# Prayforhanluo/HiCHap_master

Hardware: AMD Instinct MI355X
Metric: ICE iterations/sec on 10 kb whole-genome matrix (also nnz*iters/sec) (higher is better)
Workload: dtype f64; 1 GPU; hg19-10kb-diploid-wholegenome; n_bins=607282, nnz_upper=4998527599, resolution_bp=10000, parallelism=single GPU, entries_stored=9997055198, slots_u32=160483740, slots_u16=3332512024, payload_bytes=14837255808, tiles=88993, units=88985, hbm_bytes_matrix=15785038153

## Files before the change

hichap_master_amd/_lib.py:

```python
from __future__ import annotations

import ctypes as C
import os

_HERE = os.path.dirname(os.path.abspath(__file__))
LIB_PATH = os.environ.get("HH_LIB") or os.path.join(_HERE, "libhichap_hip.so")

HH_OK = 0


class HipLibraryError(RuntimeError):

    def __init__(self, code, msg):
        super().__init__(f"[hh rc={code}] {msg}")
        self.code = code


class MatrixInfo(C.Structure):
    _fields_ = [(n, C.c_int64) for n in (
        "n_bins", "row_lo", "row_hi", "nnz_upper", "n_entries", "n_slots", "n_tiles",
        "n_units", "n_wide", "device_bytes", "n_slots_narrow", "payload_bytes")] + [
        (n, C.c_int32) for n in ("n_chroms", "ignore_diags", "cis_only", "device", "band_w", "n_units_flat")] + [
        ("n_band", C.c_int64), ("payload_bytes_flat", C.c_int64)] + [
        (n, C.c_int32) for n in ("band_w4", "upper")]
# ... 31 lines not shown
    "hh_ktime_query": (C.c_int, [C.c_char_p, P, P]),
    "hh_ktime_reset": (C.c_int, []),
    "hh_matrix_from_pixels": (C.c_int, [P, P, P, I64, I64, P, I32, I32, I32, I64, I64, P, C.POINTER(P)]),
    "hh_matrix_from_pixels_device": (C.c_int, [P, P, P, I64, I64, P, I32, I32, I32, I64, I64, P, C.POINTER(P)]),
    "hh_matrix_free": (C.c_int, [P]),
    "hh_matrix_get_info": (C.c_int, [P, C.POINTER(MatrixInfo)]),
    "hh_matrix_export_upper": (C.c_int, [P, P, P, P, PI64]),
    "hh_synth_count": (C.c_int, [C.POINTER(SynthParams), P, P, P]),
    "hh_synth_build": (C.c_int, [C.POINTER(SynthParams), I64, I64, P, C.POINTER(P)]),
    "hh_synth_dense": (C.c_int, [P, I32, P, P]),
    "hh_synth_pixels": (C.c_int, [C.POINTER(SynthParams), I32, P, C.POINTER(P)]),
    "hh_pixels_get": (C.c_int, [P, P, P, P, PI64]),
    "hh_pixels_free": (C.c_int, [P]),
    "hh_ice_balance": (C.c_int, [P, C.POINTER(IceOpts), P, P, P, P, P, PF64, P]),
    "hh_ice_create": (C.c_int, [P, C.POINTER(IceOpts), C.POINTER(P)]),
    "hh_ice_free": (C.c_int, [P]),
    "hh_ice_n_groups": (C.c_int, [P, PI32]),
    "hh_ice_marg_local": (C.c_int, [P, I32, P, P]),
    "hh_ice_set_marg": (C.c_int, [P, P, I32, I64, P, P]),
    "hh_ice_filter_nnz": (C.c_int, [P, P]),
    "hh_ice_filter_count_mad": (C.c_int, [P, P]),
    "hh_ice_update": (C.c_int, [P, P]),
    "hh_ice_active_groups": (C.c_int, [P, PI32, P]),
    "hh_ice_iterations_done": (C.c_int, [P, PI32]),
    "hh_ice_run": (C.c_int, [P, I32, P]),
    "hh_ice_finalize": (C.c_int, [P, P, P, P, P, P, P]),
    "hh_ice_last_sweep_timing": (C.c_int, [P, PF64, PI32, PF64]),
    "hh_ice_swept_bytes": (C.c_int, [P, PI64]),
    "hh_ice_get_bias": (C.c_int, [P, P, P]),
    "hh_ice_set_bias": (C.c_int, [P, P, P]),
    "hh_ice_uband_fallbacks": (C.c_int, [P, PI64, P]),
    "hh_sweep_trace": (C.c_int, [P, I64, PI64]),
    "hh_matrix_stream_probe": (C.c_int, [P, I32, PF64, I32]),
    "hh_comm_unique_id": (C.c_int, [P]),
    "hh_comm_init": (C.c_int, [P, I32, I32, C.POINTER(P)]),
    "hh_comm_free": (C.c_int, [P]),
    "hh_comm_allgather": (C.c_int, [P, I64, P, P, P]),
    "hh_comm_reduce_scatter": (C.c_int, [P, I64, P, P, P]),
    "hh_ice_set_column_exchange": (C.c_int, [P, I32, I32, P, P, P, P, P]),
    "hh_ice_balance_sharded": (C.c_int, [P, C.POINTER(IceOpts), I32, I32, P, P, P, P, P, P, P, P, PF64, P]),
    "hh_ice_balance_cis_local": (C.c_int, [P, C.POINTER(IceOpts), I32, I64, P, P, P, P, P, P, P, PF64, P]),
    "hh_ice_filters_sharded": (C.c_int, [P, I32, P, P, P, P]),
    "hh_ice_run_sharded": (C.c_int, [P, I32, P, P, P, I32, P]),
    "hh_dense_rowstats": (C.c_int, [P, I32, I64, P, P, P, P, I32, P]),
    "hh_dense_symvc": (C.c_int, [P, I32, I64, P, P, F64, F64, P, I32, P]),
    "hh_twostep": (C.c_int, [P, P, P, I64, P, P, P, P, I32, P]),
    "hh_twostep_batch": (C.c_int, [I32, P, P, P, P, P, P, P, P, I32, P]),
    "hh_dense_from_cells": (C.c_int, [P, P, P, I64, I64, I64, I32, I32, P, P]),
    "hh_dense_upper_count": (C.c_int, [P, I64, PI64, P]),
    "hh_dense_upper_write": (C.c_int, [P, I64, P, P, P, P]),
    "hh_comp_create": (C.c_int, [P, I64, I32, P, C.POINTER(P)]),
    "hh_comp_free": (C.c_int, [P]),
    "hh_comp_colnnz": (C.c_int, [P, P, P]),
    "hh_comp_diag_sums": (C.c_int, [P, P, P, P]),
    "hh_comp_sliding_oe": (C.c_int, [P, P, I32, P]),
    "hh_comp_get_sliding_oe": (C.c_int, [P, P, P]),
    "hh_comp_correlation": (C.c_int, [P, P, P, I64, P]),
    "hh_comp_get_cor": (C.c_int, [P, P, P]),
    "hh_comp_set_cor": (C.c_int, [P, P, P]),
    "hh_gap_scan": (C.c_int, [P, I64, I32, I32, P, I32, P]),
    "hh_di_scan": (C.c_int, [P, I64, I32, P, P, I32, P, I32, P]),
    "hh_band_from_pixels": (C.c_int, [P, P, P, I64, P, I64, I64, I64, I32, P, I32, P]),
    "hh_tad_scan_pixels": (C.c_int, [P, P, P, I64, P, I64, I64, I64, I32, P, I32, P, P, I32, P]),
    "hh_viterbi_gmm": (C.c_int, [P, I64, I32, I32, P, P, P, P, P, P, P]),
    "hh_hmm_bw_create": (C.c_int, [P, P, I64, I32, I32, P, C.POINTER(P)]),
    "hh_hmm_bw_free": (C.c_int, [P]),
# ... 112 lines not shown
```

hichap_master_amd/csrc/ice.hip:

```cpp
#include <algorithm>
#include <chrono>
#include <functional>
#include <cmath>
#include <limits>

#include "ice_internal.hpp"

namespace hh {
constexpr int kThreads = 256;

constexpr int kSweepThreads = 512;
constexpr int kSweepWaves = kSweepThreads / 64;
constexpr int kFlatU = 8;
static_assert(kFlatU == kFlatIlvU, "k_sweep_flatw walks the interleaved layout's runs");

__device__ __forceinline__ double lds_b(const double* bl, uint32_t byteoff) {
    return *reinterpret_cast<const double*>(reinterpret_cast<const char*>(bl) + byteoff);
}

__device__ __forceinline__ void tile_dot(const uint4 v, const double* __restrict__ bl, double& a0, double& a1) {
    const uint32_t w[4] = {v.x, v.y, v.z, v.w};
    double x[4];
#pragma unroll
    for (int i = 0; i < 4; ++i) x[i] = lds_b(bl, w[i] & 0xFFFFu);
// ... 904 lines not shown
            flat_seg<UW, ABL, 4, true>(payw4, vw, qaw, qbw, i0w, i1w, fstw, fidw, nfw, bl, acc, lane, ca);
        } else {
            flat_seg_c<U, ABL, 8>(payn4, v, qan, qbn, i0n, i1n, fstn, nfn, bl, accc, lane);
            flat_seg<UW, ABL, 4>(payw4, vw, qaw, qbw, i0w, i1w, fstw, fidw, nfw, bl, acc, lane);
        }
        if (defer) {
            nfn_prev = nfn;
            fidn_prev = reinterpret_cast<const uint16_t*>(rg) + 2 * (kR + 1);
        } else {
            __syncthreads();
            for (int k = threadIdx.x; k < nfn; k += kSweepThreads) acc[fidn[k]] += accc[k];
        }
    }
    __syncthreads();
    for (int k = threadIdx.x; k < nfn_prev; k += kSweepThreads) acc[fidn_prev[k]] += accc[k];
    if (UP && cslot >= 0) flush_cols(L.cacc, T.colpart + (size_t)cslot * kW, kSweepThreads);
    __syncthreads();
    for (int k = threadIdx.x; k < nr; k += kSweepThreads) part[T.u_slot[u] + k] = acc[k];
}

template <int U, int ABL, bool UP>
__global__ __launch_bounds__(kSweepThreads, 4) void k_sweep_flat(TileDev T, const uint8_t* __restrict__ act,
                                                               int n_list, int list_off,
                                                               const double* __restrict__ b, long long n_bins,
                                                               double* __restrict__ part) {
    __shared__ __attribute__((aligned(16))) FlatLds<UP> L;
    if ((int)blockIdx.x >= n_list) return;
    sweep_flat_unit<U, ABL, UP>(T, act, T.u_order[list_off + blockIdx.x], b, n_bins, part, L);
}


template <int NW, bool UP>
struct FlatWLds {
    double bl[kW];
    u64 cacc[UP ? kW : 1];
    uint16_t rec[NW][kFrecU4 * 8];
    double acc[NW][kR];
    int next;
};

__device__ __forceinline__ void wave_lds_sync() {
    __builtin_amdgcn_fence(__ATOMIC_RELEASE, "wavefront");
    __builtin_amdgcn_wave_barrier();
    __builtin_amdgcn_fence(__ATOMIC_ACQUIRE, "wavefront");
}


template <int U, int ABL, int PIPE = 2, int NW = kFlatWaves, bool UP = false>
__global__ __launch_bounds__(NW * 64, NW > 8 ? 3 : 2) void k_sweep_flatw(TileDev T, const uint8_t* __restrict__ act,
                                                                       const double* __restrict__ b, long long n_bins,
                                                                       double* __restrict__ part) {
    constexpr int UW = 2;
    __shared__ __attribute__((aligned(16))) FlatWLds<NW, UP> L;
    const int k0 = T.fg_ptr[blockIdx.x], nk = T.fg_ptr[blockIdx.x + 1] - k0;
    {
        bool on = false;
        for (int k = 0; k < nk && !on; ++k) {
            const int u = T.fg_unit[k0 + k];
            for (int g = T.u_glo[u]; g <= T.u_ghi[u]; ++g) on |= act[g] != 0;
        }
        if (!on) return;
    }
    const int wave = __builtin_amdgcn_readfirstlane(threadIdx.x >> 6), lane = threadIdx.x & 63;
    const int J = T.tile_J[T.u_tlo[T.fg_unit[k0]]];
    const FlatDesc* __restrict__ desc = T.fg_desc + k0;
    const int cslot = UP && T.upper ? T.fg_cslot[blockIdx.x] : -1;
    if (threadIdx.x == 0) L.next = 0;
    if (ABL != 2 && threadIdx.x < kSweepThreads) stage_bias(L.bl, b, (long long)J * kW, n_bins);
    if (cslot >= 0)
        for (int k = threadIdx.x; k < kW; k += NW * 64) L.cacc[k] = 0;
    __syncthreads();
    const double* __restrict__ bl = L.bl;
    uint16_t* __restrict__ rec = L.rec[wave];
    double* __restrict__ acc = L.acc[wave];
    const uint16_t* fstn = rec;
    const uint16_t* fstw = rec + (kR + 1);
    const uint16_t* fidn = rec + 2 * (kR + 1);
    const uint16_t* fidw = fidn + kR;
    struct Tw {
        int slot, frec, nr, nfn, nfw;
        uint32_t qbn, qbw;
        const uint4 *payn4, *payw4;
        int up;
        const u64* bblk;
    };
    auto grab = [&](Tw& x) -> bool {
        for (;;) {
            int k = 0;
            if (lane == 0) k = atomicAdd(&L.next, 1);
            k = __builtin_amdgcn_readfirstlane(__shfl(k, 0, 64));
            if (k >= nk) return false;
            const FlatDesc d = desc[k];
            bool on = false;
            const int ngr = d.ghi - d.glo + 1;
            if (ngr <= 64) {
                const uint8_t a = act[d.glo + (lane < ngr ? lane : ngr - 1)];
                on = __ballot((a != 0) & (lane < ngr)) != 0;
            } else {
                for (int g = d.glo; g <= d.ghi; ++g) on |= act[g] != 0;
            }
            if (!on) continue;
            x = Tw{d.slot, d.frec, (int)d.nr, (int)d.nfn, (int)d.nfw, d.qbn, d.qbw,
                   reinterpret_cast<const uint4*>(T.payn + d.entn), reinterpret_cast<const uint4*>(T.pay + d.ent),
                   cslot >= 0 && d.upper ? 1 : 0, T.bfix + T.row_lo + (long long)d.rb * kR};
            return true;
        }
    };
    Tw cur;
    const bool any = grab(cur);
    uint4 v[U], vw[UW];
    if (any && cur.nfn) flat_load_ilv<U>(cur.payn4, 0u, cur.qbn, lane, v);
    if (any && cur.nfw) flat_load<UW>(cur.payw4, (uint32_t)lane * UW, 0u, cur.qbw, vw);
    for (; any;) {
        const uint4* rg = T.frec + (size_t)cur.frec * kFrecU4;
        const bool idn = cur.nfn == cur.nr;
        {
            static_assert((kR + 1 + 7) / 8 + 1 <= 2 * 64, "record range > 2 uint4 per lane");
            uint4* r4 = reinterpret_cast<uint4*>(rec);
            const int h0[4] = {0, kR + 1, 2 * (kR + 1), 2 * (kR + 1) + kR};
            const int h1[4] = {cur.nfn + 1, kR + 1 + cur.nfw + 1, idn ? 2 * (kR + 1) : 2 * (kR + 1) + cur.nfn,
                               2 * (kR + 1) + kR + cur.nfw};
            uint4 tq[4][2];
            int qs[4][2];
#pragma unroll
            for (int g = 0; g < 4; ++g) {
                const int q0 = h0[g] / 8, q1 = (h1[g] + 7) / 8;
#pragma unroll
                for (int h = 0; h < 2; ++h) {
                    const int q = q0 + lane + 64 * h;
                    qs[g][h] = q < q1 ? q : q0;
                    tq[g][h] = rg[qs[g][h]];
                }
            }
#pragma unroll
            for (int g = 0; g < 4; ++g)
#pragma unroll
                for (int h = 0; h < 2; ++h) r4[qs[g][h]] = tq[g][h];
        }
        wave_lds_sync();
        const ColArgs ca{cur.bblk, L.cacc};
        if (UP && cur.up) {
            flat_seg_c<U, ABL, 8, true, true>(cur.payn4, v, 0u, cur.qbn, 0, cur.nfn, fstn, cur.nfn, bl, acc, lane,
                                              ca, idn ? nullptr : fidn);
        } else {
            if (PIPE)
                flat_seg_c_pipe<U, ABL, 8, false, true>(cur.payn4, v, 0u, cur.qbn, 0, cur.nfn, fstn, cur.nfn, bl, acc,
                                                        lane);
            else
                flat_seg_c<U, ABL, 8, false, true>(cur.payn4, v, 0u, cur.qbn, 0, cur.nfn, fstn, cur.nfn, bl, acc, lane);
        }
        wave_lds_sync();
        constexpr int PL = kR / 64;
        double cv[PL];
        int cid[PL];
#pragma unroll
        for (int q = 0; q < PL; ++q) {
            const int i = lane + 64 * q;
            cv[q] = i < cur.nfn ? acc[i] : 0.0;
            cid[q] = i < cur.nfn ? (idn ? i : (int)fidn[i]) : -1;
        }
        wave_lds_sync();
#pragma unroll
        for (int q = 0; q < PL; ++q) acc[lane + 64 * q] = 0.0;
        wave_lds_sync();
#pragma unroll
        for (int q = 0; q < PL; ++q)
            if (cid[q] >= 0) acc[cid[q]] = cv[q];
        wave_lds_sync();
        if (UP && cur.up) {
            if (PIPE)
                flat_seg_pipe<UW, ABL, 4, true>(cur.payw4, vw, 0u, cur.qbw, 0, cur.nfw, fstw, fidw, cur.nfw, bl, acc, lane,
                                                ca);
            else flat_seg<UW, ABL, 4, true>(cur.payw4, vw, 0u, cur.qbw, 0, cur.nfw, fstw, fidw, cur.nfw, bl, acc, lane, ca);
        } else {
            if (PIPE) flat_seg_pipe<UW, ABL, 4>(cur.payw4, vw, 0u, cur.qbw, 0, cur.nfw, fstw, fidw, cur.nfw, bl, acc, lane);
            else flat_seg<UW, ABL, 4>(cur.payw4, vw, 0u, cur.qbw, 0, cur.nfw, fstw, fidw, cur.nfw, bl, acc, lane);
        }
        wave_lds_sync();
        Tw nxt;
        bool more = false;
        if (PIPE == 2) {
            more = grab(nxt);
            if (more) {
                if (nxt.nfn) flat_load_ilv<U>(nxt.payn4, 0u, nxt.qbn, lane, v);
                if (nxt.nfw) flat_load<UW>(nxt.payw4, (uint32_t)lane * UW, 0u, nxt.qbw, vw);
            }
        }
        double* __restrict__ out = part + cur.slot;
        for (int r = lane; r < cur.nr; r += 64) out[r] = acc[r];
        wave_lds_sync();
        if (PIPE != 2) {
            more = grab(nxt);
            if (more) {
                if (nxt.nfn) flat_load_ilv<U>(nxt.payn4, 0u, nxt.qbn, lane, v);
                if (nxt.nfw) flat_load<UW>(nxt.payw4, (uint32_t)lane * UW, 0u, nxt.qbw, vw);
            }
        }
        if (!more) break;
        cur = nxt;
    }
    if (UP && cslot >= 0) {
// ... 1169 lines not shown
    DBuf<unsigned long long> cx_send, cx_recv, cx_all;
    int32_t iters_done = 0;
    PinnedBuf<uint8_t> h_active;
    std::vector<hipEvent_t> ev;
    double sweep_ms = 0.0, iter_ms = 0.0;
    int32_t sweep_launches = 0;
    hipStream_t side = nullptr, side2 = nullptr;
    hipEvent_t fork = nullptr, join = nullptr, join2 = nullptr;
    ~hh_ice() {
        for (auto e : ev) (void)hipEventDestroy(e);
        if (join2) (void)hipEventDestroy(join2);
        if (side2) (void)hipStreamDestroy(side2);
        if (fork) (void)hipEventDestroy(fork);
        if (join) (void)hipEventDestroy(join);
        if (side) (void)hipStreamDestroy(side);
    }
    bool full() const { return m->row_lo == 0 && m->row_hi == m->n_bins; }
    TileArgs ta() {
        return TileArgs{tile_lo.p, tile_hi.p, tile_group.p, group_tile_ptr.p, blk_tile_ptr.p, tile_cnt.p,
                        tile_sum.p, tile_sq.p, g_cnt.p, g_sum.p, counter.p};
    }
    bool small_stats() const { return hh::g_fuse_stats == 1 || (hh::g_fuse_stats < 0 && n_tiles <= hh::kFuseMaxTiles); }
    uint8_t* act() { return active.p + (iters_done & 1) * G; }
    uint8_t* nxt() { return active.p + (1 - (iters_done & 1)) * G; }
};

namespace hh {

static int g_sweep_nb = 2;
static int g_band_dpp = 0;
static int g_flatw_waves = 11;
static int g_flatw_waves_up = 8;
static int g_flatw_pipe = 2;
static int g_sweep_ablate = 0;
static int g_tiled_pf = 1;
static int g_band_concurrent = 1;
static int g_split_tiles = 1;
static int g_conc_order = 1;
static int64_t g_conc_min_bytes = 8LL << 30;
static int64_t g_conc_ub_min_bytes = 1LL << 30;
static int g_band_rows = 0;
static int g_band_fused = 1;
static int g_band_lpt = 1;
static int g_uband = 1;
static int64_t g_uband_min_bytes = 128LL << 20;
static int g_ub_xcd = 1;
static int g_ub_fast = 1;
static int g_sweep_single = -1;
static int g_iter_events = 1;
static int64_t g_single_max_bytes = 1LL << 30;
static unsigned long long* g_trace = nullptr;
static int64_t g_trace_cap = 0, g_trace_n = 0;

template <int NB, int ABL, bool UP>
static void launch_sweep_up(const hh_matrix* m, const TileDev& T, const uint8_t* act, const double* b, double* part,
                            hipStream_t s, hipStream_t s_tiled, int which) {
    const int n_tiled = (int)(m->n_units - m->n_units_flat), n_flat = (int)m->n_units_flat;
    auto tiled = [&] {
        if (!n_tiled) return;
        HH_KTIME("k_sweep_tiled", s_tiled);
        auto kern = k_sweep_tiled<NB, ABL, UP>;
        if constexpr (NB == 2 && ABL <= 2 && !UP) {
            if (g_tiled_pf == 1) kern = k_sweep_tiled<NB, ABL, UP, 1>;
            if constexpr (ABL == 0)
                if (g_tiled_pf == 2) kern = k_sweep_tiled<NB, ABL, UP, 2>;
        }
        hipLaunchKernelGGL(kern, dim3((unsigned)n_tiled), dim3(kSweepThreads), 0, s_tiled, T, act, n_tiled, b,
                           (long long)m->n_bins, part);
    };
    if (which & 1) tiled();
    if (!(which & 2)) return;
    HH_KTIME(n_flat ? "k_sweep_flat" : nullptr, s);
    if (n_flat && m->n_fgroups) {
        HH_REQUIRE(m->flat_perm, "column-grouped flat tiles without the interleaved layout");
        auto kern = g_flatw_pipe == 2   ? k_sweep_flatw<kFlatU, ABL, 2>
                    : g_flatw_pipe == 1 ? k_sweep_flatw<kFlatU, ABL, 1>
                                        : k_sweep_flatw<kFlatU, ABL, 0>;
        int nw = 8;
        if constexpr (UP) {
            nw = g_flatw_waves_up == 11 ? 11 : 8;
            kern = nw == 11 ? k_sweep_flatw<kFlatU, ABL, 2, 11, true> : k_sweep_flatw<kFlatU, ABL, 2, 8, true>;
        } else {
            if (g_flatw_waves == 10) {
                kern = g_flatw_pipe == 2 ? k_sweep_flatw<kFlatU, ABL, 2, 10> : k_sweep_flatw<kFlatU, ABL, 0, 10>;
                nw = 10;
            } else if (g_flatw_waves == 11) {
                kern = g_flatw_pipe == 2 ? k_sweep_flatw<kFlatU, ABL, 2, 11> : k_sweep_flatw<kFlatU, ABL, 0, 11>;
                nw = 11;
            }
        }
        hipLaunchKernelGGL(kern, dim3((unsigned)m->n_fgroups), dim3(64 * nw), 0, s, T, act, b,
                           (long long)m->n_bins, part);
    } else if (n_flat) {
        hipLaunchKernelGGL((k_sweep_flat<kFlatU, ABL, UP>), dim3((unsigned)n_flat), dim3(kSweepThreads), 0, s, T,
                           act, n_flat, n_tiled, b, (long long)m->n_bins, part);
    }
}

template <int NB, int ABL>
static void launch_sweep(const hh_matrix* m, const TileDev& T, const uint8_t* act, const double* b, double* part,
                         hipStream_t s, hipStream_t s_tiled, int which) {
    if constexpr (kUpperBuild) {
        if (T.upper) return launch_sweep_up<NB, ABL, true>(m, T, act, b, part, s, s_tiled, which);
    }
    launch_sweep_up<NB, ABL, false>(m, T, act, b, part, s, s_tiled, which);
}

template <int ABL>
static void launch_sweep_nb(const hh_matrix* m, const TileDev& T, const uint8_t* act, const double* b, double* part,
                            hipStream_t s, hipStream_t st, int which) {
    switch (g_sweep_nb) {
        case 1: launch_sweep<1, ABL>(m, T, act, b, part, s, st, which); break;
        case 2: launch_sweep<2, ABL>(m, T, act, b, part, s, st, which); break;
        case 8: launch_sweep<8, ABL>(m, T, act, b, part, s, st, which); break;
        default: launch_sweep<4, ABL>(m, T, act, b, part, s, st, which); break;
    }
}

static void sweep(const hh_matrix* m, const TileDev& T, const uint8_t* act, const double* b, double* part,
                  hipStream_t s, hipStream_t s_tiled = nullptr, int which = 3) {
    if (m->n_units == 0) return;
    if (!s_tiled) s_tiled = s;
    switch (g_sweep_ablate) {
        case 1: launch_sweep_nb<1>(m, T, act, b, part, s, s_tiled, which); break;
        case 2: launch_sweep_nb<2>(m, T, act, b, part, s, s_tiled, which); break;
// ... 325 lines not shown
    const double med = np_median(logm);
    std::vector<double> dev(logm.size());
    for (size_t k = 0; k < logm.size(); ++k) dev[k] = std::fabs(logm[k] - med);
    const double cutoff = std::exp(med - S->o.mad_max * np_median(dev));
    for (int64_t i = 0; i < S->n; ++i)
        if (marg[i] < cutoff) bias[i] = 0.0;
    upload_pinned_sync(S->bias.p, bias.data(), (size_t)S->n, s);
}

extern "C" {

int hh_tune(const char* key, int64_t value) {
    return guard([&] {
        HH_REQUIRE(key, "null key");
        const std::string k(key);
        if (k == "sweep_nb") {
            HH_REQUIRE(value == 1 || value == 2 || value == 4 || value == 8, "sweep_nb must be 1, 2, 4 or 8");
            g_sweep_nb = (int)value;
        } else if (k == "tiled_pf") {
            HH_REQUIRE(value >= 0 && value <= 2, "tiled_pf in {0, 1, 2}");
            g_tiled_pf = (int)value;
        } else if (k == "sweep_ablate") {
            HH_REQUIRE(value >= 0 && value <= 3, "sweep_ablate must be 0, 1, 2 or 3");
            g_sweep_ablate = (int)value;
        } else if (k == "band4_density_pct" || k == "band8_big_pct") {
            HH_REQUIRE(value >= 1 && value <= 100, "percent in [1, 100]");
            (k == "band4_density_pct" ? g_band4_density : g_band8_big) = (double)value / 100.0;
        } else if (k == "band4") {
            HH_REQUIRE(value == 0 || value == 1, "band4 in {0, 1}");
            g_band4 = value;
        } else if (k == "flat_cols") {
            HH_REQUIRE(value >= -1 && value <= 1, "flat_cols in {-1 (auto), 0, 1}");
            g_flat_cols = value;
        } else if (k == "flatw_pipe") {
            HH_REQUIRE(value >= 0 && value <= 2, "flatw_pipe in {0, 1, 2}");
            g_flatw_pipe = (int)value;
        } else if (k == "band_dpp") {
            HH_REQUIRE(value == 0 || value == 1, "band_dpp in {0, 1}");
            g_band_dpp = (int)value;
        } else if (k == "flatw_u") {
            HH_REQUIRE(value == 8, "flatw_u: 8 (the interleaved flat layout's run length)");
        } else if (k == "flatw_waves_up") {
            HH_REQUIRE(value == 8 || value == 11, "flatw_waves_up in {8, 11}");
            g_flatw_waves_up = (int)value;
        } else if (k == "upper_tiles") {
            HH_REQUIRE(value >= -1 && value <= 1, "upper_tiles in {-1 (auto), 0, 1}");
            HH_REQUIRE(kUpperBuild || value != 1,
                       "upper-triangle tiles need the 4096-column build (libhichap_hip_up.so, -DHH_KWBITS=12)");
            g_upper_tiles = value;
        } else if (k == "flat_max") {
            HH_REQUIRE(value >= 0 && value <= 255, "flat_max in [0, 255]");
            g_flat_max = value;
        } else if (k == "unit_entries") {
            HH_REQUIRE(value == 0 || (value >= 4096 && value <= (1 << 24)), "unit_entries must be 0 (auto) or in [4096, 2^24]");
            g_unit_entries = value;
        } else if (k == "flat_defer") {
            HH_REQUIRE(value == 0 || value == 1, "flat_defer in {0, 1}");
            g_flat_defer = (int)value;
        } else if (k == "unit_lpt") {
            HH_REQUIRE(value >= 0 && value <= 2, "unit_lpt in {0, 1, 2}");
            g_unit_lpt = value;
        } else if (k == "unit_lpt_lists") {
            HH_REQUIRE(value >= 0 && value <= 3, "unit_lpt_lists in [0, 3]");
            g_unit_lpt_lists = value;
        } else if (k == "tile_cost") {
            HH_REQUIRE(value >= 0 && value <= (1 << 20), "tile_cost in [0, 2^20] payload words");
// ... 727 lines not shown
```

hichap_master_amd/csrc/matrix.hip:

```cpp
#include <algorithm>
#include <atomic>
#include <chrono>
#include <cstdio>
#include <cmath>
#include <numeric>
#include <exception>
#include <mutex>
#include <thread>

#include "ice_internal.hpp"

namespace hh {

static thread_local std::string g_last_error;
int64_t g_unit_entries = 0;
int g_flat_defer = 1;
int64_t g_unit_lpt = 1;
int64_t g_unit_lpt_lists = 1;
int64_t g_flat_group = 0;
int64_t g_flat_cols = -1;
bool flat_cols_on(int32_t nJ) { return g_flat_cols > 0 || (g_flat_cols < 0 && nJ >= 32); }
int64_t g_tile_cost = 32768;
int64_t g_band_w = -1;
int64_t g_flat_max = 64;
// ... 501 lines not shown
    m.u_tlo = to_device(P.u_tlo, s);
    m.u_thi = to_device(P.u_thi, s);
    m.u_rb = to_device(P.u_rb, s);
    m.u_rlo = to_device(P.u_rlo, s);
    m.u_rhi = to_device(P.u_rhi, s);
    m.u_slot = to_device(P.u_slot, s);
    m.u_glo = to_device(P.u_glo, s);
    m.u_ghi = to_device(P.u_ghi, s);
    m.blk_unit_ptr = to_device(P.blk_unit_ptr, s);
    m.u_order = to_device(P.u_order, s);
    m.tile_perm = to_device(P.tile_perm, s);
    m.tile_band = to_device(P.tile_band, s);
    m.tile_fw = to_device(P.tile_fw, s);
    m.tile_frec = to_device(P.tile_frec, s);
    m.frec = to_device(P.frec, s);
    m.u_whole = to_device(P.u_whole, s);
    m.n_fgroups = P.fg_ptr.empty() ? 0 : (int64_t)P.fg_ptr.size() - 1;
    if (m.n_fgroups) {
        m.fg_ptr = to_device(P.fg_ptr, s);
        m.fg_unit = to_device(P.fg_unit, s);
        m.fg_desc = to_device(P.fg_desc, s);
    }
    m.upper = P.upper;
    m.n_cslots = P.n_cslots;
    if (P.upper) {
        m.u_cslot = to_device(P.u_cslot, s);
        if (!P.fg_cslot.empty()) m.fg_cslot = to_device(P.fg_cslot, s);
        m.jslot_ptr = to_device(P.jslot_ptr, s);
        if (!P.jslot.empty()) m.jslot = to_device(P.jslot, s);
    }
    HIP_CHECK(hipStreamSynchronize(s));
}

}

using namespace hh;

extern "C" {

const char* hh_last_error(void) { return g_last_error.c_str(); }
int hh_version(void) { return (0 << 16) | (2 << 8) | 0; }

int hh_ktime_enable(int32_t on) {
    return guard([&] { hh::g_ktime_on = on != 0; });
}

int hh_ktime_query(const char* name, double* total_ms, int64_t* calls) {
    return guard([&] {
        HH_REQUIRE(name && total_ms && calls, "bad arguments");
        std::lock_guard<std::mutex> lk(hh::g_ktime_mu);
        double t = 0.0;
        int64_t c = 0;
        for (auto& r : hh::g_ktime) {
            if (std::strcmp(r.name, name) != 0) continue;
            HIP_CHECK(hipEventSynchronize(r.b));
            float ms = 0.f;
            HIP_CHECK(hipEventElapsedTime(&ms, r.a, r.b));
            t += ms;
            ++c;
        }
        *total_ms = t;
        *calls = c;
    });
}

int hh_ktime_reset(void) {
    return guard([&] {
        std::lock_guard<std::mutex> lk(hh::g_ktime_mu);
        for (auto& r : hh::g_ktime) {
            (void)hipEventSynchronize(r.b);
            (void)hipEventDestroy(r.a);
// ... 357 lines not shown
```

hichap_master_amd/ice.py:

```python
from __future__ import annotations

import ctypes as C
from dataclasses import asdict, dataclass

import numpy as np

from . import _lib
from ._lib import IceOpts, MatrixInfo, SynthParams, call, ptr


@dataclass
class IceOptions:
    ignore_diags: int = 1
    cis_only: bool = False
    mad_max: int = 5
    min_nnz: int = 10
    min_count: float = 0
    tol: float = 1e-5
    max_iters: int = 200
    rescale_marginals: bool = True
    check_every: int = 8

    def c_opts(self) -> IceOpts:
        return IceOpts(int(self.mad_max), int(self.min_nnz), float(self.min_count), float(self.tol),
                       int(self.max_iters), int(bool(self.rescale_marginals)),
                       int(self.check_every), 0)


class ContactMatrix:

    def __init__(self, handle, chrom_offsets):
        self._h = handle
        self.chrom_offsets = np.asarray(chrom_offsets, dtype=np.int64)

    @classmethod
    def from_pixels(cls, bin1, bin2, count, n_bins, chrom_offsets, ignore_diags=1,
                    cis_only=False, row_range=None, stream=None):
        _lib.require_gpu()
        b1 = np.ascontiguousarray(bin1, dtype=np.int64)
        b2 = np.ascontiguousarray(bin2, dtype=np.int64)
        cnt = np.ascontiguousarray(count, dtype=np.float64)
# ... 27 lines not shown
        call("hh_matrix_from_pixels_device", p1, p2, pc, int(n), int(n_bins), ptr(off), off.size - 1,
             int(ignore_diags), int(bool(cis_only)), lo, hi, stream, C.byref(h))
        return cls(h, off)

    @classmethod
    def synthetic(cls, chrom_nbins, row_range=None, stream=None, **kw):
        _lib.require_gpu()
        p, keep = synth_params(chrom_nbins, **kw)
        n = int(np.sum(chrom_nbins))
        lo, hi = (0, n) if row_range is None else (int(row_range[0]), int(row_range[1]))
        h = C.c_void_p()
        call("hh_synth_build", C.byref(p), lo, hi, stream, C.byref(h))
        off = np.concatenate([[0], np.cumsum(chrom_nbins)]).astype(np.int64)
        return cls(h, off)

    @property
    def handle(self):
        return self._h

    def info(self) -> dict:
        inf = MatrixInfo()
        call("hh_matrix_get_info", self._h, C.byref(inf))
        return {k: getattr(inf, k) for k, _ in MatrixInfo._fields_}

    def export_upper(self):
        n = C.c_int64(0)
        call("hh_matrix_export_upper", self._h, None, None, None, C.byref(n))
        b1 = np.empty(n.value, np.int64)
        b2 = np.empty(n.value, np.int64)
        c = np.empty(n.value, np.float64)
        call("hh_matrix_export_upper", self._h, ptr(b1), ptr(b2), ptr(c), C.byref(n))
        return b1, b2, c

    def close(self):
        if self._h:
            call("hh_matrix_free", self._h)
            self._h = None

    def __del__(self):
        try:
            self.close()
        except Exception:
            pass


def synth_params(chrom_nbins, A=30.0, decay=1.08, comp_strength=0.3, vis_sigma=0.3, gap_frac=0.02,
                 trans_density=0.0, comp_block=200, ignore_diags=1, cis_only=False, seed=20201015):
    arr = np.ascontiguousarray(chrom_nbins, dtype=np.int32)
    p = SynthParams(arr.size, arr.ctypes.data_as(C.POINTER(C.c_int32)), float(A), float(decay),
                    float(comp_strength), float(vis_sigma), float(gap_frac), float(trans_density),
                    int(comp_block), int(ignore_diags), int(bool(cis_only)), 0, int(seed))
    return p, arr


class DevArray:

    def __init__(self, p, n, owner=None):
        self._p, self._n, self._owner = int(p or 0), int(n), owner

    def data_ptr(self):
        return self._p

    def numel(self):
        return self._n


# ... 185 lines not shown
```

include/hichap_hip.h:

```cpp
#ifndef HICHAP_HIP_H
#define HICHAP_HIP_H

#include <stdint.h>

#ifdef __cplusplus
extern "C" {
#endif

#define HH_OK 0
#define HH_ERR_ARG -1
#define HH_ERR_HIP -2
#define HH_ERR_OOM -3
#define HH_ERR_STATE -4

const char* hh_last_error(void);
int hh_version(void);
int hh_device_count(int32_t* n);
int hh_set_device(int32_t device);
int hh_synchronize(void* stream);
int hh_device_copy(void* dst, const void* src, int64_t bytes, void* stream);
int hh_tune(const char* key, int64_t value);
int hh_sweep_trace(uint64_t* out, int64_t cap, int64_t* n);
int hh_ktime_enable(int32_t on);
int hh_ktime_query(const char* name, double* total_ms, int64_t* calls);
// ... 5 lines not shown
    int64_t n_bins;
    int64_t row_lo, row_hi;
    int64_t nnz_upper;
    int64_t n_entries;
    int64_t n_slots;
    int64_t n_tiles;
    int64_t n_units;
    int64_t n_wide;
    int64_t device_bytes;
    int64_t n_slots_narrow;
    int64_t payload_bytes;
    int32_t n_chroms;
    int32_t ignore_diags;
    int32_t cis_only;
    int32_t device;
    int32_t band_w;
    int32_t n_units_flat;
    int64_t n_band;
    int64_t payload_bytes_flat;
    int32_t band_w4;
    int32_t upper;
} hh_matrix_info;

int hh_matrix_from_pixels(const int64_t* bin1, const int64_t* bin2, const double* count,
                          int64_t nnz, int64_t n_bins, const int64_t* chrom_offsets,
                          int32_t n_chroms, int32_t ignore_diags, int32_t cis_only,
                          int64_t row_lo, int64_t row_hi, void* stream, hh_matrix** out);
int hh_matrix_from_pixels_device(const int32_t* bin1, const int32_t* bin2, const int32_t* count, int64_t nnz,
                                 int64_t n_bins, const int64_t* chrom_offsets, int32_t n_chroms, int32_t ignore_diags,
                                 int32_t cis_only, int64_t row_lo, int64_t row_hi, void* stream, hh_matrix** out);
int hh_matrix_free(hh_matrix* m);
int hh_matrix_get_info(const hh_matrix* m, hh_matrix_info* info);
int hh_matrix_stream_probe(const hh_matrix* m, int32_t reps, double* out, int32_t nout);
int hh_matrix_export_upper(const hh_matrix* m, int64_t* bin1, int64_t* bin2, double* count,
                           int64_t* nnz_inout);

typedef struct {
    int32_t n_chroms;
    const int32_t* chrom_nbins;
    double A;
    double decay;
    double comp_strength;
    double vis_sigma;
    double gap_frac;
    double trans_density;
    int32_t comp_block;
    int32_t ignore_diags;
    int32_t cis_only;
    int32_t pad_;
    uint64_t seed;
} hh_synth_params;

int hh_synth_count(const hh_synth_params* p, int32_t* row_work, int64_t* row_nnz_upper,
                   void* stream);
int hh_synth_dense(const hh_synth_params* p, int32_t chrom, double* out, void* stream);
typedef struct hh_pixels hh_pixels;
int hh_synth_pixels(const hh_synth_params* p, int32_t ordered, void* stream, hh_pixels** out);
int hh_pixels_get(const hh_pixels* P, const int32_t** bin1, const int32_t** bin2, const int32_t** count, int64_t* nnz);
int hh_pixels_free(hh_pixels* P);
int hh_synth_build(const hh_synth_params* p, int64_t row_lo, int64_t row_hi, void* stream,
                   hh_matrix** out);

typedef struct {
    int32_t mad_max;
    int32_t min_nnz;
    double min_count;
// ... 184 lines not shown
```

Measured before the change: 341.9 ICE iterations/s.

## Stage flat-group descriptors and activity flags in LDS; skip identity compaction

```diff
diff --git a/hichap_master_amd/_lib.py b/hichap_master_amd/_lib.py
--- a/hichap_master_amd/_lib.py
+++ b/hichap_master_amd/_lib.py
@@ -87,6 +87,8 @@
     "hh_ice_uband_fallbacks": (C.c_int, [P, PI64, P]),
     "hh_sweep_trace": (C.c_int, [P, I64, PI64]),
     "hh_matrix_stream_probe": (C.c_int, [P, I32, PF64, I32]),
+    "hh_matrix_flat_audit": (C.c_int, [P, I32, P]),
+    "hh_flat_audit_plan": (C.c_int, [P, I64, P, P, I64, P, P, P]),
     "hh_comm_unique_id": (C.c_int, [P]),
     "hh_comm_init": (C.c_int, [P, I32, I32, C.POINTER(P)]),
     "hh_comm_free": (C.c_int, [P]),
diff --git a/hichap_master_amd/csrc/ice.hip b/hichap_master_amd/csrc/ice.hip
--- a/hichap_master_amd/csrc/ice.hip
+++ b/hichap_master_amd/csrc/ice.hip
@@ -960,12 +960,19 @@
 
 template <int NW, bool UP>
 struct FlatWLds {
+    static constexpr int kStage = NW > 8 ? 48 : 256;
     double bl[kW];
     u64 cacc[UP ? kW : 1];
     uint16_t rec[NW][kFrecU4 * 8];
     double acc[NW][kR];
+    FlatDesc desc[kStage];
+    uint8_t on[kStage];
     int next;
 };
+static_assert(sizeof(FlatWLds<11, false>) <= 163840 && sizeof(FlatWLds<10, false>) <= 163840 &&
+                  sizeof(FlatWLds<8, false>) <= 163840 &&
+                  (!kUpperBuild || (sizeof(FlatWLds<11, true>) <= 163840 && sizeof(FlatWLds<8, true>) <= 163840)),
+              "k_sweep_flatw: one block's LDS is at most the CU's 160 KB");
 
 __device__ __forceinline__ void wave_lds_sync() {
     __builtin_amdgcn_fence(__ATOMIC_RELEASE, "wavefront");
@@ -973,15 +980,22 @@
     __builtin_amdgcn_fence(__ATOMIC_ACQUIRE, "wavefront");
 }
 
+__device__ __forceinline__ uint32_t wave_u32(uint32_t x) { return (uint32_t)__builtin_amdgcn_readfirstlane((int)x); }
+__device__ __forceinline__ long long wave_i64(long long x) {
+    const uint32_t lo = wave_u32((uint32_t)x), hi = wave_u32((uint32_t)((unsigned long long)x >> 32));
+    return (long long)(((unsigned long long)hi << 32) | lo);
+}
+
 
 template <int U, int ABL, int PIPE = 2, int NW = kFlatWaves, bool UP = false>
 __global__ __launch_bounds__(NW * 64, NW > 8 ? 3 : 2) void k_sweep_flatw(TileDev T, const uint8_t* __restrict__ act,
                                                                        const double* __restrict__ b, long long n_bins,
-                                                                       double* __restrict__ part) {
+                                                                       double* __restrict__ part, int chain) {
     constexpr int UW = 2;
     __shared__ __attribute__((aligned(16))) FlatWLds<NW, UP> L;
     const int k0 = T.fg_ptr[blockIdx.x], nk = T.fg_ptr[blockIdx.x + 1] - k0;
-    {
+    const bool staged = chain && nk <= FlatWLds<NW, UP>::kStage;
+    if (!staged) {
         bool on = false;
         for (int k = 0; k < nk && !on; ++k) {
             const int u = T.fg_unit[k0 + k];
@@ -994,10 +1008,22 @@
     const FlatDesc* __restrict__ desc = T.fg_desc + k0;
     const int cslot = UP && T.upper ? T.fg_cslot[blockIdx.x] : -1;
     if (threadIdx.x == 0) L.next = 0;
+    if (staged && (int)threadIdx.x < nk) {
+        const FlatDesc d = desc[threadIdx.x];
+        bool on = false;
+        for (int g = d.glo; g <= d.ghi; ++g) on |= act[g] != 0;
+        L.desc[threadIdx.x] = d;
+        L.on[threadIdx.x] = on ? 1 : 0;
+    }
     if (ABL != 2 && threadIdx.x < kSweepThreads) stage_bias(L.bl, b, (long long)J * kW, n_bins);
     if (cslot >= 0)
         for (int k = threadIdx.x; k < kW; k += NW * 64) L.cacc[k] = 0;
     __syncthreads();
+    if (staged) {
+        bool on = false;
+        for (int k = threadIdx.x & 63; k < nk; k += 64) on |= L.on[k] != 0;
+        if (__ballot(on) == 0) return;
+    }
     const double* __restrict__ bl = L.bl;
     uint16_t* __restrict__ rec = L.rec[wave];
     double* __restrict__ acc = L.acc[wave];
@@ -1018,6 +1044,17 @@
             if (lane == 0) k = atomicAdd(&L.next, 1);
             k = __builtin_amdgcn_readfirstlane(__shfl(k, 0, 64));
             if (k >= nk) return false;
+            if (staged) {
+                if (wave_u32(L.on[k]) == 0) continue;
+                const FlatDesc& d = L.desc[k];
+                const long long entn = wave_i64(d.entn), ent = wave_i64(d.ent);
+                x = Tw{(int)wave_u32((uint32_t)d.slot), (int)wave_u32((uint32_t)d.frec), (int)wave_u32(d.nr),
+                       (int)wave_u32(d.nfn), (int)wave_u32(d.nfw), wave_u32(d.qbn), wave_u32(d.qbw),
+                       reinterpret_cast<const uint4*>(T.payn + entn), reinterpret_cast<const uint4*>(T.pay + ent),
+                       cslot >= 0 && wave_u32(d.upper) ? 1 : 0,
+                       T.bfix + T.row_lo + (long long)wave_u32(d.rb) * kR};
+                return true;
+            }
             const FlatDesc d = desc[k];
             bool on = false;
             const int ngr = d.ghi - d.glo + 1;
@@ -1078,23 +1115,25 @@
                 flat_seg_c<U, ABL, 8, false, true>(cur.payn4, v, 0u, cur.qbn, 0, cur.nfn, fstn, cur.nfn, bl, acc, lane);
         }
         wave_lds_sync();
-        constexpr int PL = kR / 64;
-        double cv[PL];
-        int cid[PL];
-#pragma unroll
-        for (int q = 0; q < PL; ++q) {
-            const int i = lane + 64 * q;
-            cv[q] = i < cur.nfn ? acc[i] : 0.0;
-            cid[q] = i < cur.nfn ? (idn ? i : (int)fidn[i]) : -1;
-        }
-        wave_lds_sync();
-#pragma unroll
-        for (int q = 0; q < PL; ++q) acc[lane + 64 * q] = 0.0;
-        wave_lds_sync();
-#pragma unroll
-        for (int q = 0; q < PL; ++q)
-            if (cid[q] >= 0) acc[cid[q]] = cv[q];
-        wave_lds_sync();
+        if (!(chain && idn)) {
+            constexpr int PL = kR / 64;
+            double cv[PL];
+            int cid[PL];
+#pragma unroll
+            for (int q = 0; q < PL; ++q) {
+                const int i = lane + 64 * q;
+                cv[q] = i < cur.nfn ? acc[i] : 0.0;
+                cid[q] = i < cur.nfn ? (idn ? i : (int)fidn[i]) : -1;
+            }
+            wave_lds_sync();
+#pragma unroll
+            for (int q = 0; q < PL; ++q) acc[lane + 64 * q] = 0.0;
+            wave_lds_sync();
+#pragma unroll
+            for (int q = 0; q < PL; ++q)
+                if (cid[q] >= 0) acc[cid[q]] = cv[q];
+            wave_lds_sync();
+        }
         if (UP && cur.up) {
             if (PIPE)
                 flat_seg_pipe<UW, ABL, 4, true>(cur.payw4, vw, 0u, cur.qbw, 0, cur.nfw, fstw, fidw, cur.nfw, bl, acc, lane,
@@ -2330,6 +2369,7 @@
 static int g_flatw_waves = 11;
 static int g_flatw_waves_up = 8;
 static int g_flatw_pipe = 2;
+static int g_flat_chain = 1;
 static int g_sweep_ablate = 0;
 static int g_tiled_pf = 1;
 static int g_band_concurrent = 1;
@@ -2388,7 +2428,7 @@
             }
         }
         hipLaunchKernelGGL(kern, dim3((unsigned)m->n_fgroups), dim3(64 * nw), 0, s, T, act, b,
-                           (long long)m->n_bins, part);
+                           (long long)m->n_bins, part, g_flat_chain);
     } else if (n_flat) {
         hipLaunchKernelGGL((k_sweep_flat<kFlatU, ABL, UP>), dim3((unsigned)n_flat), dim3(kSweepThreads), 0, s, T,
                            act, n_flat, n_tiled, b, (long long)m->n_bins, part);
@@ -2780,6 +2820,9 @@
         } else if (k == "flat_cols") {
             HH_REQUIRE(value >= -1 && value <= 1, "flat_cols in {-1 (auto), 0, 1}");
             g_flat_cols = value;
+        } else if (k == "flat_chain") {
+            HH_REQUIRE(value == 0 || value == 1, "flat_chain in {0, 1}");
+            g_flat_chain = (int)value;
         } else if (k == "flatw_pipe") {
             HH_REQUIRE(value >= 0 && value <= 2, "flatw_pipe in {0, 1, 2}");
             g_flatw_pipe = (int)value;
diff --git a/hichap_master_amd/csrc/matrix.hip b/hichap_master_amd/csrc/matrix.hip
--- a/hichap_master_amd/csrc/matrix.hip
+++ b/hichap_master_amd/csrc/matrix.hip
@@ -557,11 +557,173 @@
     HIP_CHECK(hipStreamSynchronize(s));
 }
 
+namespace {
+struct FlatAudit {
+    int64_t* out;
+    bool bad = false;
+    void fail(int64_t tile, int field, int64_t index, int64_t size) {
+        if (bad) return;
+        bad = true;
+        out[0] = 1;
+        out[1] = tile;
+        out[2] = field;
+        out[3] = index;
+        out[4] = size;
+    }
+    void in(int64_t tile, int field, int64_t i, int64_t n) {
+        if (i < 0 || i >= n) fail(tile, field, i, n);
+    }
+};
+}
+
+bool flat_audit_plan(const FlatDesc* desc, int64_t n_desc, const int32_t* fg_ptr, const int32_t* fg_J,
+                     int64_t n_fgroups, const uint16_t* frec, const int64_t* sizes, int64_t* out) {
+    enum { kDesc = 1, kAct, kFrec, kPayn, kPay, kPart, kBias, kBfix, kRecord };
+    const int64_t n_act = sizes[0], n_frec4 = sizes[1], n_payn4 = sizes[2] / 8, n_pay4 = sizes[3] / 4,
+                  n_part = sizes[4], n_bins = sizes[5], n_bfix = sizes[6], row_lo = sizes[7];
+    for (int i = 0; i < HH_FLAT_AUDIT_NOUT; ++i) out[i] = 0;
+    FlatAudit A{out};
+    constexpr uint32_t kStep = 64u * kFlatIlvU;
+    for (int64_t g = 0; g < n_fgroups; ++g) {
+        const int64_t k0 = fg_ptr[g], k1 = fg_ptr[g + 1];
+        if (k0 < 0 || k1 < k0) A.fail(-1 - g, kDesc, k0, n_desc);
+        if (k1 > k0) {
+            A.in(k0, kDesc, k0, n_desc);
+            A.in(k1 - 1, kDesc, k1 - 1, n_desc);
+        }
+        if (A.bad) break;
+        out[8] = std::max<int64_t>(out[8], k1 - k0);
+        if (fg_J) {
+            const int64_t c0 = (int64_t)fg_J[g] * kW;
+            A.in(-1 - g, kBias, c0, n_bins);
+        }
+        for (int64_t k = k0; k < k1; ++k) {
+            const FlatDesc& d = desc[k];
+            const bool idn = d.nfn == d.nr;
+            ++out[idn ? 5 : 6];
+            if (d.nr < kR) ++out[7];
+            A.in(k, kAct, d.glo, n_act);
+            A.in(k, kAct, d.ghi, n_act);
+            if (d.ghi < d.glo) A.fail(k, kAct, (int64_t)d.glo - 1, n_act);
+            if (d.nr < 1 || d.nr > kR) A.fail(k, kRecord, d.nr, kR);
+            if (d.nfn > d.nr) A.fail(k, kRecord, d.nfn, d.nr);
+            if (d.nfw > d.nr) A.fail(k, kRecord, d.nfw, d.nr);
+            if (d.frec < 0) A.fail(k, kFrec, d.frec, n_frec4 / kFrecU4);
+            const int64_t r0 = (int64_t)d.frec * kFrecU4;
+            const int h0[4] = {0, kR + 1, 2 * (kR + 1), 2 * (kR + 1) + kR};
+            const int h1[4] = {d.nfn + 1, kR + 1 + d.nfw + 1, idn ? 2 * (kR + 1) : 2 * (kR + 1) + d.nfn,
+                               2 * (kR + 1) + kR + d.nfw};
+            for (int q = 0; q < 4; ++q) {
+                const int q0 = h0[q] / 8, q1 = (h1[q] + 7) / 8;
+                A.in(k, kFrec, r0 + q0, n_frec4);
+                if (q1 > q0) A.in(k, kFrec, r0 + q1 - 1, n_frec4);
+                if (q1 > kFrecU4) A.fail(k, kFrec, q1 - 1, kFrecU4);
+                if (q1 - q0 > 2 * 64) A.fail(k, kFrec, q0 + 2 * 64, q1);
+            }
+            if (d.entn < 0 || d.entn % 8) A.fail(k, kPayn, d.entn, sizes[2]);
+            const int64_t pn = d.entn / 8;
+            if (d.nfn) {
+                if (!d.qbn) A.fail(k, kPayn, pn, n_payn4);
+                for (uint32_t q0 = 0; q0 < d.qbn && !A.bad; q0 += kStep) {
+                    const uint32_t m = std::min(d.qbn - q0, kStep);
+                    uint32_t base = q0;
+                    A.in(k, kPayn, pn + q0, n_payn4);
+                    for (int e = 0; e < kFlatIlvU; ++e) {
+                        const uint32_t cnt = flat_ilv_cnt(m, e);
+                        if (cnt) {
+                            if (base + cnt > d.qbn) A.fail(k, kPayn, pn + base + cnt - 1, pn + d.qbn);
+                            A.in(k, kPayn, pn + base + cnt - 1, n_payn4);
+                        }
+                        base += cnt;
+                    }
+                }
+            }
+            if (d.ent < 0 || d.ent % 4) A.fail(k, kPay, d.ent, sizes[3]);
+            const int64_t pw = d.ent / 4;
+            if (d.nfw) {
+                if (!d.qbw) A.fail(k, kPay, pw, n_pay4);
+                A.in(k, kPay, pw, n_pay4);
+                if (d.qbw) A.in(k, kPay, pw + d.qbw - 1, n_pay4);
+            }
+            A.in(k, kPart, d.slot, n_part);
+            A.in(k, kPart, (int64_t)d.slot + d.nr - 1, n_part);
+            if (n_bfix > 0 && d.upper) {
+                A.in(k, kBfix, row_lo + (int64_t)d.rb * kR, n_bfix);
+                A.in(k, kBfix, row_lo + (int64_t)d.rb * kR + d.nr - 1, n_bfix);
+            }
+            if (frec && !A.bad) {
+                const uint16_t* r = frec + (size_t)r0 * 8;
+                const uint16_t *fstn = r, *fstw = r + (kR + 1), *fidn = r + 2 * (kR + 1), *fidw = fidn + kR;
+                for (int i = 0; i < d.nfn; ++i)
+                    if (fstn[i] > fstn[i + 1]) A.fail(k, kRecord, fstn[i], fstn[i + 1]);
+                if (fstn[d.nfn] != d.qbn) A.fail(k, kRecord, fstn[d.nfn], d.qbn);
+                for (int i = 0; i < d.nfw; ++i)
+                    if (fstw[i] > fstw[i + 1]) A.fail(k, kRecord, fstw[i], fstw[i + 1]);
+                if (fstw[d.nfw] != d.qbw) A.fail(k, kRecord, fstw[d.nfw], d.qbw);
+                for (int i = 0; i < d.nfn; ++i)
+                    if (fidn[i] >= d.nr || (idn && fidn[i] != i)) A.fail(k, kRecord, fidn[i], d.nr);
+                for (int i = 0; i < d.nfw; ++i)
+                    if (fidw[i] >= d.nr) A.fail(k, kRecord, fidw[i], d.nr);
+            }
+            if (A.bad) break;
+        }
+        if (A.bad) break;
+    }
+    out[9] = n_desc;
+    out[10] = n_fgroups;
+    return !A.bad;
+}
+
 }
 
 using namespace hh;
 
 extern "C" {
+
+int hh_flat_audit_plan(const void* desc, int64_t n_desc, const int32_t* fg_ptr, const int32_t* fg_J,
+                       int64_t n_fgroups, const uint16_t* frec, const int64_t* sizes, int64_t* out) {
+    return guard([&] {
+        HH_REQUIRE(fg_ptr && sizes && out && (desc || !n_desc) && n_desc >= 0 && n_fgroups >= 0, "null");
+        if (!flat_audit_plan(static_cast<const FlatDesc*>(desc), n_desc, fg_ptr, fg_J, n_fgroups, frec, sizes, out))
+            HH_THROW(HH_ERR_STATE, "flat plan audit: tile " + std::to_string(out[1]) + " field " +
+                                       std::to_string(out[2]) + " index " + std::to_string(out[3]) +
+                                       " outside a buffer of " + std::to_string(out[4]));
+    });
+}
+
+int hh_matrix_flat_audit(const hh_matrix* m, int32_t n_groups, int64_t* out) {
+    return guard([&] {
+        HH_REQUIRE(m && out && n_groups >= 1, "null");
+        HIP_CHECK(hipSetDevice(m->device));
+        for (int i = 0; i < HH_FLAT_AUDIT_NOUT; ++i) out[i] = 0;
+        if (!m->n_fgroups) return;
+        std::vector<int32_t> ptr((size_t)m->n_fgroups + 1), unit(m->fg_unit.n), tlo(m->u_tlo.n), tJ(m->tile_J.n);
+        std::vector<FlatDesc> desc(m->fg_desc.n);
+        std::vector<uint16_t> frec(m->frec.n);
+        m->fg_ptr.download(ptr.data(), ptr.size(), 0);
+        m->fg_unit.download(unit.data(), unit.size(), 0);
+        m->u_tlo.download(tlo.data(), tlo.size(), 0);
+        m->tile_J.download(tJ.data(), tJ.size(), 0);
+        m->fg_desc.download(desc.data(), desc.size(), 0);
+        m->frec.download(frec.data(), frec.size(), 0);
+        HIP_CHECK(hipDeviceSynchronize());
+        std::vector<int32_t> J((size_t)m->n_fgroups, 0);
+        for (int64_t g = 0; g < m->n_fgroups; ++g) {
+            const int64_t k0 = ptr[g];
+            HH_REQUIRE(k0 >= 0 && k0 < (int64_t)unit.size() && unit[k0] >= 0 && unit[k0] < (int64_t)tlo.size() &&
+                           tlo[unit[k0]] >= 0 && tlo[unit[k0]] < (int64_t)tJ.size(),
+                       "flat plan audit: a group's first unit or tile is outside the plan");
+            J[g] = tJ[tlo[unit[k0]]];
+        }
+        const int64_t sizes[8] = {n_groups, (int64_t)(m->frec.n / 8), (int64_t)m->payn.n, (int64_t)m->pay.n,
+                                  std::max<int64_t>(m->n_part, 1), m->n_bins, m->upper ? m->n_bins : 0, m->row_lo};
+        if (!flat_audit_plan(desc.data(), (int64_t)desc.size(), ptr.data(), J.data(), m->n_fgroups, frec.data(), sizes,
+                             out))
+            HH_THROW(HH_ERR_STATE, "flat plan audit: tile " + std::to_string(out[1]) + " field " +
+                                       std::to_string(out[2]) + " index " + std::to_string(out[3]) +
+                                       " outside a buffer of " + std::to_string(out[4]));
+    });
+}
 
 const char* hh_last_error(void) { return g_last_error.c_str(); }
 int hh_version(void) { return (0 << 16) | (2 << 8) | 0; }
diff --git a/hichap_master_amd/ice.py b/hichap_master_amd/ice.py
--- a/hichap_master_amd/ice.py
+++ b/hichap_master_amd/ice.py
@@ -6,7 +6,40 @@
 import numpy as np
 
 from . import _lib
-from ._lib import IceOpts, MatrixInfo, SynthParams, call, ptr
+from ._lib import HipLibraryError, IceOpts, MatrixInfo, SynthParams, call, ptr
+
+FLAT_DESC = np.dtype([("entn", "<i8"), ("ent", "<i8"), ("frec", "<i4"), ("slot", "<i4"), ("qbn", "<u4"),
+                      ("qbw", "<u4"), ("nr", "<u2"), ("nfn", "<u2"), ("nfw", "<u2"), ("glo", "<u2"),
+                      ("ghi", "<u2"), ("upper", "<u2"), ("rb", "<u4")])
+FLAT_AUDIT_NOUT = 16
+FLAT_AUDIT_FIELDS = (None, "desc", "act", "frec", "payn", "pay", "part", "bias", "bfix", "record")
+
+
+def _audit_dict(out):
+    v = None
+    if out[0]:
+        v = {"tile": int(out[1]), "field": FLAT_AUDIT_FIELDS[int(out[2])], "index": int(out[3]),
+             "size": int(out[4])}
+    return {"ok": not out[0], "violation": v, "idn": int(out[5]), "not_idn": int(out[6]),
+            "short_blocks": int(out[7]), "max_group": int(out[8]), "tiles": int(out[9]), "groups": int(out[10])}
+
+
+def flat_audit_plan(desc, fg_ptr, sizes, fg_J=None, frec=None) -> dict:
+    desc = np.ascontiguousarray(desc, dtype=FLAT_DESC)
+    fg_ptr = np.ascontiguousarray(fg_ptr, dtype=np.int32)
+    sizes = np.ascontiguousarray(sizes, dtype=np.int64)
+    if sizes.shape != (8,):
+        raise ValueError("flat_audit_plan: eight sizes")
+    fg_J = None if fg_J is None else np.ascontiguousarray(fg_J, dtype=np.int32)
+    frec = None if frec is None else np.ascontiguousarray(frec, dtype=np.uint16)
+    out = np.zeros(FLAT_AUDIT_NOUT, np.int64)
+    try:
+        call("hh_flat_audit_plan", ptr(desc), desc.size, ptr(fg_ptr), ptr(fg_J), fg_ptr.size - 1, ptr(frec),
+             ptr(sizes), ptr(out))
+    except HipLibraryError:
+        if not out[0]:
+            raise
+    return _audit_dict(out)
 
 
 @dataclass
@@ -100,6 +133,15 @@
         call("hh_matrix_export_upper", self._h, ptr(b1), ptr(b2), ptr(c), C.byref(n))
         return b1, b2, c
 
+    def flat_audit(self, n_groups: int) -> dict:
+        out = np.zeros(FLAT_AUDIT_NOUT, np.int64)
+        try:
+            call("hh_matrix_flat_audit", self._h, int(n_groups), ptr(out))
+        except HipLibraryError:
+            if not out[0]:
+                raise
+        return _audit_dict(out)
+
     def close(self):
         if self._h:
             call("hh_matrix_free", self._h)
diff --git a/include/hichap_hip.h b/include/hichap_hip.h
--- a/include/hichap_hip.h
+++ b/include/hichap_hip.h
@@ -61,6 +61,10 @@
 int hh_matrix_free(hh_matrix* m);
 int hh_matrix_get_info(const hh_matrix* m, hh_matrix_info* info);
 int hh_matrix_stream_probe(const hh_matrix* m, int32_t reps, double* out, int32_t nout);
+#define HH_FLAT_AUDIT_NOUT 16
+int hh_matrix_flat_audit(const hh_matrix* m, int32_t n_groups, int64_t* out);
+int hh_flat_audit_plan(const void* desc, int64_t n_desc, const int32_t* fg_ptr, const int32_t* fg_J,
+                       int64_t n_fgroups, const uint16_t* frec, const int64_t* sizes, int64_t* out);
 int hh_matrix_export_upper(const hh_matrix* m, int64_t* bin1, int64_t* bin2, double* count,
                            int64_t* nnz_inout);
 
```

Measured after the change: 345.3 ICE iterations/s, median of 6. 1.0% higher.
